# samuel-vitorino/lm.rs

Hardware: AMD Instinct MI355X
Metric: decode tok/s + %HBM-roofline, Llama-3.2-1B Q8_0 @1/2/4/8 MI355X vs CPU ref (higher is better)
Workload: dtype int8xint8->int32, f32 combine; 1 GPU; llama-3.2-1b Q8_0 (gs=128) greedy decode, 5-token synthetic prompt then 3164 tokens, batch 1; parallelism=single GPU, image_bytes=1274634496

## Files before the change

### lm.rs_amd/csrc/lmrs_kernels.hip

```cpp
#include <hip/hip_ext.h>
#include <mutex>
#include <map>
#include <set>
#include <tuple>
#include <utility>

#include "lmrs_device_math.h"
#include "lmrs_kernels.h"
#include "lmrs_stage.h"

namespace lmrs {

constexpr int kBlock = 256;
constexpr int kGS = 128;


constexpr int kMaxP = 16;

template <int NP>
__device__ __forceinline__ void rmsnorm_inplace(float4 (&v)[NP], const float4 (&wv)[NP], int n, float eps,
                                                int add_unit, float* scratch) {
    const int t = threadIdx.x;
    const int P = (n + 1023) >> 10;
    const int JP = (n >> 3) + 4;
// ... 805 lines not shown
    int best = cl;
    for (int L = cl; L <= maxL; L *= 2) {
        const int NC = L / cl;
        if (G % NC) continue;
        const int Gc = G / NC;
        if (NC > 1 && Gc > 16) continue;
        best = L;
        const int RB = (64 / L) * (kBlock / 64);
        if ((a.o + RB - 1) / RB >= 256) break;
    }
    const int NC = best / cl, Gc = G / NC;
    const int U = NC == 1 ? 16 : (Gc <= 4 ? 4 : (Gc <= 8 ? 8 : 16));
    return {best, U, NP};
}

#define LMRS_GEMV_TABLE(X)                                                                                 \
                                                                                              \
    X(8, 16, 10, PRO_PREQ, EPI_STORE, false) X(8, 16, 10, PRO_QUANT, EPI_STORE, false) X(8, 16, 10, PRO_QUANT, EPI_RESID, false) X(8, 16, 10, PRO_PREQ, EPI_RESID, false) \
    X(8, 16, 10, PRO_RMS_QUANT, EPI_STORE, false) X(8, 16, 10, PRO_RMS_QUANT, EPI_QKV, false)              \
    X(8, 16, 10, PRO_RMS_QUANT, EPI_SWIGLU, false) X(8, 16, 10, PRO_RMS_QUANT, EPI_GELU, false) X(8, 16, 10, PRO_RMS_QUANT, EPI_CLS, false) \
          \
    X(8, 16, 16, PRO_PREQ, EPI_STORE, false) X(8, 16, 16, PRO_QUANT, EPI_STORE, false) X(8, 16, 16, PRO_QUANT, EPI_RESID, false) X(8, 16, 16, PRO_PREQ, EPI_RESID, false) \
    X(4, 16, 16, PRO_PREQ, EPI_STORE, true) X(4, 16, 16, PRO_QUANT, EPI_STORE, true) X(4, 16, 16, PRO_QUANT, EPI_RESID, true) \
                                                      \
    X(32, 4, 2, PRO_RMS_QUANT, EPI_QKV, false) X(32, 4, 2, PRO_QUANT, EPI_RESID, false) X(32, 4, 2, PRO_QUANT, EPI_STORE, false) \
    X(8, 16, 2, PRO_RMS_QUANT, EPI_SWIGLU, false) X(8, 16, 2, PRO_RMS_QUANT, EPI_CLS, false) X(8, 16, 2, PRO_RMS_QUANT, EPI_QKV, false) \
    X(32, 4, 2, PRO_PREQ, EPI_STORE, false) X(8, 16, 2, PRO_PREQ, EPI_STORE, false) X(16, 8, 2, PRO_PREQ, EPI_STORE, false) \
                                              \
    X(16, 16, 4, PRO_RMS_QUANT, EPI_QKV, false) X(32, 8, 4, PRO_QUANT, EPI_RESID, false) X(16, 16, 4, PRO_QUANT, EPI_RESID, false) \
    X(8, 16, 4, PRO_RMS_QUANT, EPI_SWIGLU, false) X(8, 16, 4, PRO_RMS_QUANT, EPI_GELU, false) X(8, 16, 4, PRO_RMS_QUANT, EPI_CLS, false) \
    X(16, 16, 4, PRO_PREQ, EPI_STORE, false) X(32, 8, 4, PRO_PREQ, EPI_STORE, false)                       \
                                                                         \
    X(32, 16, 10, PRO_QUANT, EPI_RESID, false) X(32, 16, 10, PRO_QUANT, EPI_STORE, false) X(64, 16, 10, PRO_QUANT, EPI_STORE, false) \
    X(64, 16, 10, PRO_QUANT, EPI_RESID, false) X(32, 16, 10, PRO_PREQ, EPI_STORE, false) X(64, 16, 10, PRO_PREQ, EPI_STORE, false) \
                                                             \
    X(4, 16, 10, PRO_PREQ, EPI_STORE, true) X(4, 16, 10, PRO_QUANT, EPI_STORE, true) X(4, 16, 10, PRO_QUANT, EPI_RESID, true) \
    X(4, 16, 10, PRO_RMS_QUANT, EPI_STORE, true) X(4, 16, 10, PRO_RMS_QUANT, EPI_QKV, true) X(4, 16, 10, PRO_RMS_QUANT, EPI_SWIGLU, true) \
    X(4, 16, 10, PRO_RMS_QUANT, EPI_GELU, true) X(4, 16, 10, PRO_RMS_QUANT, EPI_CLS, true)                 \
    X(16, 4, 10, PRO_PREQ, EPI_STORE, true) X(16, 4, 10, PRO_QUANT, EPI_RESID, true) X(16, 4, 10, PRO_QUANT, EPI_STORE, true) \
    X(16, 4, 10, PRO_RMS_QUANT, EPI_QKV, true) X(16, 16, 10, PRO_QUANT, EPI_RESID, true) X(16, 16, 10, PRO_QUANT, EPI_STORE, true) \
    X(16, 16, 10, PRO_PREQ, EPI_STORE, true) X(8, 16, 10, PRO_PREQ, EPI_STORE, true) X(8, 16, 10, PRO_RMS_QUANT, EPI_QKV, true)

static bool gemv_instantiated(int L, int U, int NP, int pro, int epi, bool q4) {
#define X(l, u, np, p, e, q) if (L == l && U == u && NP == np && pro == p && epi == e && q4 == q) return true;
    LMRS_GEMV_TABLE(X)
#undef X
    return false;
}

static GemvShape resolve_shape(const GemvArgs& a, int pro, int epi) {
    GemvShape sh = pick_shape(a, epi);
    if (!gemv_instantiated(sh.L, sh.U, sh.NP, pro, epi, a.q4 != 0)) {
        const int big = a.n <= 10240 ? 10 : 16;
        if (gemv_instantiated(sh.L, sh.U, big, pro, epi, a.q4 != 0)) sh.NP = big;
        else sh = {a.q4 ? 4 : 8, 16, big};
    }
    return sh;
}

int gemv_grid(const GemvArgs& a, int pro, int epi) {
    const StaticClass sc = static_class(a, pro, epi);
    const GemvShape sh = sc.L ? GemvShape{sc.L, 0, 0} : resolve_shape(a, pro, epi);
    const int RB = (64 / sh.L) * ((sc.L ? sc.nt : kBlock) / 64);
    const int n_pass = (a.o + RB - 1) / RB;
    int cap = 4096;
    if (epi == EPI_CLS) cap = 512;
    else if (sc.L && (epi == EPI_SWIGLU || epi == EPI_GELU)) {
        int k = 2;
        if (n_pass / 2 > 256 && n_pass / 2 < 448 && (n_pass + 2) / 3 <= 256) k = 3;
        cap = (n_pass + k - 1) / k;
    }
    return n_pass < cap ? n_pass : cap;
}

hipError_t launch_gemv(const GemvArgs& a0, int pro, int epi, hipStream_t s, int grid_hint) {
    GemvArgs a = a0;
    a.order_barrier = a.chain_spread = 1;
    if (a.n % kGS != 0 || a.n > kMaxP * 1024 || a.o <= 0) return hipErrorInvalidValue;
    int grid = grid_hint > 0 ? grid_hint : gemv_grid(a, pro, epi);
    if (grid_hint > 0 && (epi == EPI_SWIGLU || epi == EPI_GELU)) {
        const int least = gemv_grid(a, pro, epi);
        if (grid < least) grid = least;
    }
    if (epi == EPI_CLS && a.has_tail && (!a.tail.cls_seq || !a.tail.err || !a.tail.part_pk || a.o + a.row_offset >= (1 << 20) - 1)) return hipErrorInvalidValue;
    const size_t smem = gemv_smem(a, pro);
    const StaticClass sc = static_class(a, pro, epi);
    if (sc.L) {
#define X(n_, l_, p_, e_, nt_, q_)                                                                         \
        if (a.n == n_ && sc.L == l_ && pro == p_ && epi == e_ && sc.nt == nt_ && (a.q4 != 0) == q_) {      \
            LMRS_LAUNCH_GRID((gemv_static_kernel<n_, l_, p_, e_, nt_, q_>), dim3(grid), nt_, smem, s, LMRS_HOT_OF(a), a);            \
            return hipGetLastError();                                                                      \
        }
        LMRS_STATIC_TABLE(X)
#undef X
    }
    if (pro == PRO_ADD_RMS_QUANT) return hipErrorInvalidValue;
    const GemvShape sh = resolve_shape(a, pro, epi);
#define X(l, u, np, p, e, q)                                                                               \
    if (sh.L == l && sh.U == u && sh.NP == np && pro == p && epi == e && (a.q4 != 0) == q) {              \
        LMRS_LAUNCH((gemv_kernel<l, u, np, p, e, q>), grid, smem, s, a);                                   \
        return hipGetLastError();                                                                          \
    }
    LMRS_GEMV_TABLE(X)
#undef X
    return hipErrorInvalidValue;
}

constexpr int kAttF4 = 16;

template <int HS> struct AttGeom {
    static constexpr int HS4 = HS / 4, RS = HS + 4;
    static constexpr bool ALIGNED = (kBlock % HS4 == 0) && ((16 * HS4) % kBlock == 0 || kBlock % (16 * HS4) == 0);
};
template <int HS, int NF>
__device__ __forceinline__ void att_gload(float4 (&rg)[NF], const float* __restrict__ base, int t0, int T, int CH, int kv_dim) {
    constexpr int HS4 = HS / 4;
    const int ct = (T - t0) < CH ? (T - t0) : CH, nrows = (ct + 15) & ~15, nf = nrows * HS4;
    const int r0 = (int)threadIdx.x / HS4, c4 = (int)threadIdx.x - r0 * HS4;
    const float* lane_base = base + (size_t)t0 * kv_dim + c4 * 4;
#pragma unroll
    for (int i0 = 0; i0 < NF; i0 += 4) {
        if (i0 * kBlock < nf) {
#pragma unroll
            for (int i = i0; i < i0 + 4 && i < NF; ++i) {
                int row;
                if constexpr (kBlock % HS4 == 0) row = r0 + i * (kBlock / HS4);
                else row = ((int)threadIdx.x + i * kBlock) / HS4;
                const int col4 = (kBlock % HS4 == 0) ? 0 : (((int)threadIdx.x + i * kBlock) - row * HS4 - c4) * 4;
                row = row < ct - 1 ? row : ct - 1;
                rg[i] = ld_f32x4<false>(lane_base + (size_t)row * kv_dim + col4);
            }
        }
    }
}
template <int HS, int NF, bool SCALE>
__device__ __forceinline__ void att_tstore(const float4 (&rg)[NF], float* tile, const float* rowscale, int t0, int T, int CH, int patch_t, const float* patch) {
    constexpr int HS4 = HS / 4, RS = HS + 4;
    const int ct = (T - t0) < CH ? (T - t0) : CH, nrows = (ct + 15) & ~15, nf = nrows * HS4;
    const int r0 = (int)threadIdx.x / HS4, c4 = (int)threadIdx.x - r0 * HS4;
#pragma unroll
    for (int i0 = 0; i0 < NF; i0 += 4) {
        if (i0 * kBlock < nf) {
            int row[4], col[4]; float sc[4];
#pragma unroll
            for (int u = 0; u < 4; ++u) {
                const int i = i0 + u;
                if constexpr (kBlock % HS4 == 0) { row[u] = r0 + i * (kBlock / HS4); col[u] = c4; }
                else { const int f = (int)threadIdx.x + i * kBlock; row[u] = f / HS4; col[u] = f - row[u] * HS4; }
                if constexpr (SCALE) sc[u] = rowscale[row[u] < nrows ? row[u] : nrows - 1];
            }
#pragma unroll
            for (int u = 0; u < 4; ++u) {
                const int i = i0 + u;
                if (i < NF && (AttGeom<HS>::ALIGNED || row[u] < nrows)) {
                    float4 v = rg[i];
                    if constexpr (SCALE) { v.x = sc[u] * v.x; v.y = sc[u] * v.y; v.z = sc[u] * v.z; v.w = sc[u] * v.w; }
                    *reinterpret_cast<float4*>(tile + row[u] * RS + col[u] * 4) = v;
                }
            }
        }
    }
    if (patch_t >= t0 && patch_t < t0 + ct) {
        const int fb = (patch_t - t0) * HS4, d = ((int)threadIdx.x - fb) & (kBlock - 1);
        if (d < HS4) {
            float4 v = *reinterpret_cast<const float4*>(patch + d * 4);
            if constexpr (SCALE) { const float ap = rowscale[patch_t - t0]; v.x = ap * v.x; v.y = ap * v.y; v.z = ap * v.z; v.w = ap * v.w; }
            *reinterpret_cast<float4*>(tile + (patch_t - t0) * RS + d * 4) = v;
        }
    }
}

#define ATT_STAMP(k) do { if (a.dbg && threadIdx.x == 0 && blockIdx.x == 0) a.dbg[k] = wall_clock64(); } while (0)

struct AttPre { float q0, q1, k0, k1; float2 cs; };

typedef float f32x4v __attribute__((ext_vector_type(4)));
__device__ __forceinline__ float* att_k_head(const AttnArgs& a, int kvh, int hs) {
    return a.k_cache + ((size_t)a.layer * a.n_kv_heads + kvh) * hs * (size_t)a.seq_len;
}
template <int NG>
__device__ __forceinline__ void att_kload(f32x4v (&dst)[NG], __amdgpu_buffer_rsrc_t krs, int voff, int g0, int S) {
#pragma unroll
    for (int u = 0; u < NG; ++u) {
        const auto t = __builtin_amdgcn_raw_buffer_load_b128(krs, voff, (g0 + u) * S * 16, 0);
        dst[u] = f32x4v{__uint_as_float(t[0]), __uint_as_float(t[1]), __uint_as_float(t[2]), __uint_as_float(t[3])};
    }
}
template <int NG>
__device__ __forceinline__ float att_kuse(float score, const f32x4v (&src)[NG], const float4* q4, int g0) {
#pragma unroll
    for (int u = 0; u < NG; ++u) {
        const float4 qq = q4[g0 + u];
        float pr;
        pr = qq.x * src[u].x; score = score + pr;
        pr = qq.y * src[u].y; score = score + pr;
        pr = qq.z * src[u].z; score = score + pr;
        pr = qq.w * src[u].w; score = score + pr;
    }
    return score;
}
template <int HS, int NG>
__device__ __forceinline__ float att_score_chain(f32x4v (&kk)[NG], __amdgpu_buffer_rsrc_t krs, int voff, const float* q, int S) {
    constexpr int HS4 = HS / 4;
    f32x4v kb[NG];
    float score = 0.0f;
    const float4* q4 = reinterpret_cast<const float4*>(q);
#pragma unroll
    for (int g0 = 0; g0 < HS4; g0 += 2 * NG) {
        if (g0 + NG < HS4) att_kload<NG>(kb, krs, voff, g0 + NG, S);
        score = att_kuse<NG>(score, kk, q4, g0);
        asm volatile("" : "+v"(score) : : "memory");
        if (g0 + NG < HS4) {
            if (g0 + 2 * NG < HS4) att_kload<NG>(kk, krs, voff, g0 + 2 * NG, S);
            score = att_kuse<NG>(score, kb, q4, g0 + NG);
            asm volatile("" : "+v"(score) : : "memory");
        }
    }
    return score;
}

__device__ __forceinline__ float2 rope_rotate(float v0, float v1, float fcr, float fci) {
    const float a0 = v0 * fcr, a1 = v1 * fci, b0 = v0 * fci, b1 = v1 * fcr;
    return make_float2(a0 - a1, b0 + b1);
}
__device__ __forceinline__ void k_store_pair(float* k, int S, int pos, int j, int half, float r0, float r1) {
    k[(((size_t)(j >> 2) * S + pos) << 2) + (j & 3)] = r0;
    k[(((size_t)((j + half) >> 2) * S + pos) << 2) + ((j + half) & 3)] = r1;
}
__device__ __forceinline__ float gemma_cap_window(float score, int wpos, int t) {
    score = score / 50.0f;
    score = (float)tanh((double)score);
    score = score * 50.0f;
    return score + (((unsigned)(wpos - t) <= 4096u) ? 0.0f : -2.3819763e38f);
}
template <int HS4>
__device__ __forceinline__ float tile_score(const float4* k, int ks, const float* qs) {
    constexpr int GB = 4;
    static_assert(HS4 % (2 * GB) == 0, "head size");
    const float4* q4 = reinterpret_cast<const float4*>(qs);
    auto dot = [](float score, const float4 (&q)[GB], const float4 (&kk)[GB]) __attribute__((always_inline)) {
#pragma unroll
        for (int u = 0; u < GB; ++u) {
            float pr;
            pr = q[u].x * kk[u].x; score = score + pr;
            pr = q[u].y * kk[u].y; score = score + pr;
            pr = q[u].z * kk[u].z; score = score + pr;
            pr = q[u].w * kk[u].w; score = score + pr;
        }
        return score;
    };
    float score = 0.0f;
    float4 ka[GB], qa[GB], kb[GB], qb[GB];
#pragma unroll
    for (int u = 0; u < GB; ++u) { ka[u] = k[u * ks]; qa[u] = q4[u]; }
#pragma unroll
    for (int g0 = 0; g0 < HS4; g0 += 2 * GB) {
#pragma unroll
        for (int u = 0; u < GB; ++u) { kb[u] = k[(g0 + GB + u) * ks]; qb[u] = q4[g0 + GB + u]; }
        asm volatile("" : "+v"(score) : : "memory");
        score = dot(score, qa, ka);
        if (g0 + 2 * GB < HS4) {
#pragma unroll
            for (int u = 0; u < GB; ++u) { ka[u] = k[(g0 + 2 * GB + u) * ks]; qa[u] = q4[g0 + 2 * GB + u]; }
        }
        asm volatile("" : "+v"(score) : : "memory");
        score = dot(score, qb, kb);
    }
    return score;
}
struct AttTag { const unsigned long long* gran; unsigned tag; int att_dim, kv_dim; int* err; };
template <int NG>
__device__ __forceinline__ void poll_granules(const unsigned long long* const (&gp)[NG], const AttTag& tg, int layer, unsigned long long (&xg)[NG]) {
    auto sweep = [&](unsigned long long (&x)[NG]) __attribute__((always_inline)) {
#pragma unroll
        for (int k = 0; k < NG; ++k) x[k] = __hip_atomic_load(gp[k], __ATOMIC_RELAXED, __HIP_MEMORY_SCOPE_AGENT);
    };
    auto fresh = [&](const unsigned long long (&x)[NG]) __attribute__((always_inline)) {
        bool ok = true;
#pragma unroll
        for (int k = 0; k < NG; ++k) ok = ok && (unsigned)(x[k] >> 32) == tg.tag;
        return __all(ok) != 0;
    };
    auto take = [&](const unsigned long long (&x)[NG]) __attribute__((always_inline)) {
#pragma unroll
        for (int k = 0; k < NG; ++k) xg[k] = x[k];
    };
    unsigned long long xa[NG], xb[NG];
    sweep(xa);
    for (unsigned spins = 0;; ++spins) {
        sweep(xb);
        if (fresh(xa)) { take(xa); break; }
        sweep(xa);
        if (fresh(xb)) { take(xb); break; }
        if (spins > kTagSpinMax || (spins & 1023) == 1023) {
            const int e = __hip_atomic_load(tg.err, __ATOMIC_RELAXED, __HIP_MEMORY_SCOPE_AGENT);
            if (e != 0 || spins > kTagSpinMax) {
                if (e == 0) __hip_atomic_store(tg.err, layer + 1, __ATOMIC_RELAXED, __HIP_MEMORY_SCOPE_AGENT);
                take(xb);
                break;
            }
        }
    }
}
__device__ __forceinline__ void granules_of(const AttTag& tg, int h, int kvh, int hs, int d, const unsigned long long** gp) {
    gp[0] = tg.gran + h * hs + d; gp[1] = tg.gran + tg.att_dim + kvh * hs + d; gp[2] = tg.gran + tg.att_dim + tg.kv_dim + kvh * hs + d;
}

template <int HS, int NF, bool COH, bool PRE = false, bool GEMMA = false, bool ROT = false, bool TAG = false>
__device__ __forceinline__ void attention_body(const AttnArgs& a, int h, int pos, char* smem, uint64_t etab, const AttPre& pre = AttPre(), const AttTag& tg = AttTag()) {
    static_assert(!PRE || HS / 2 <= kBlock, "one RoPE pair per lane");
    static_assert(!TAG || (HS <= kBlock && !COH && !PRE && !ROT), "granule polling: one value of each vector per lane");
    constexpr int half = HS / 2, RS = HS + 4;
    const int kv_mul = a.n_heads / a.n_kv_heads, kvh = h / kv_mul;
    const int kv_dim = a.n_kv_heads * HS;
    const int T = pos + 1;
    const int tid = threadIdx.x;
    const int CH = a.chunk;
    float* q = reinterpret_cast<float*>(smem);
    float* kn = q + HS;
    float* vn = kn + HS;
    float* red = vn + HS;
    float* tile = red + 16;
    float* att = tile + (size_t)(CH + 32) * RS;
    const size_t loff = (size_t)a.layer * a.seq_len * kv_dim;
    const int nchunks = (T + CH - 1) / CH;
    const float* vbase = a.v_cache + loff + kvh * HS;
    const int S = a.seq_len;
    float* kT = att_k_head(a, kvh, HS);
    const __amdgpu_buffer_rsrc_t krs = __builtin_amdgcn_make_buffer_rsrc(kT, 0, HS * S * 4, 0x00020000);
    constexpr int KG = HS / 4 <= 32 ? HS / 4 : 16;
    static_assert((HS / 4) % KG == 0, "head size");
    const int tc0 = tid < T ? tid : T - 1;
    f32x4v kk[KG];
    att_kload<KG>(kk, krs, tc0 * 16, 0, S);
    float4 vreg[NF];
    att_gload<HS, NF>(vreg, vbase, 0, T, CH, kv_dim);

    if constexpr (ROT) { for (int j = tid; j < HS; j += kBlock) q[j] = a.q[h * HS + j]; }
    float2 cs_tag = make_float2(0.f, 0.f);
    if constexpr (TAG) {
        cs_tag = *reinterpret_cast<const float2*>(a.rope + ((size_t)pos * half + (tid < half ? tid : 0)) * 2);
        if (tid < HS) {
            const unsigned long long* gp[3];
            unsigned long long xg[3];
            granules_of(tg, h, kvh, HS, tid, gp);
            poll_granules<3>(gp, tg, a.layer, xg);
            q[tid] = __uint_as_float((unsigned)xg[0]); kn[tid] = __uint_as_float((unsigned)xg[1]); vn[tid] = __uint_as_float((unsigned)xg[2]);
        }
        lds_barrier();
        ATT_STAMP(1);
    }
    for (int j = tid; j < (ROT ? 0 : half); j += kBlock) {
        float2 cs;
        if constexpr (PRE) cs = pre.cs; else if constexpr (TAG) cs = cs_tag; else cs = *reinterpret_cast<const float2*>(a.rope + ((size_t)pos * half + j) * 2);
        const float fcr = cs.x, fci = cs.y;
        const float q0 = TAG ? q[j] : PRE ? pre.q0 : ld_f32<COH>(a.q + h * HS + j), q1 = TAG ? q[j + half] : PRE ? pre.q1 : ld_f32<COH>(a.q + h * HS + j + half);
        const float2 rq = rope_rotate(q0, q1, fcr, fci);
        q[j] = rq.x; q[j + half] = rq.y;
        const float k0 = TAG ? kn[j] : PRE ? pre.k0 : ld_f32<COH>(a.k_raw + kvh * HS + j), k1 = TAG ? kn[j + half] : PRE ? pre.k1 : ld_f32<COH>(a.k_raw + kvh * HS + j + half);
        const float2 rk = rope_rotate(k0, k1, fcr, fci);
        kn[j] = rk.x; kn[j + half] = rk.y;
        k_store_pair(kT, S, pos, j, half, rk.x, rk.y);
        if constexpr (COH) {
            vn[j] = ld_f32<true>(vbase + (size_t)pos * kv_dim + j);
            vn[j + half] = ld_f32<true>(vbase + (size_t)pos * kv_dim + j + half);
        }
    }
    if (!TAG || HS / 4 > KG || T > kBlock) asm volatile("s_waitcnt vmcnt(0)" ::: "memory");
    lds_barrier();
    ATT_STAMP(2);
    if (!ROT && tc0 == pos) {
#pragma unroll
        for (int u = 0; u < KG; ++u) { const float4 t4 = reinterpret_cast<const float4*>(kn)[u]; kk[u] = f32x4v{t4.x, t4.y, t4.z, t4.w}; }
    }

    int wpos = pos;
    if constexpr (GEMMA) { const int wb = a.st->win_base; wpos = wb >= 0 ? wb : pos; }
    const float sqrt_hs = sqrtf((float)HS);
    float lmax = __uint_as_float(0xff800000u);
    auto finish_score = [&](float score, int t) __attribute__((always_inline)) {
        score = score / sqrt_hs;
        if constexpr (GEMMA) score = gemma_cap_window(score, wpos, t);
        if (t < T) { att[t] = score; lmax = fmaxf(lmax, score); }
    };
    finish_score(att_score_chain<HS, KG>(kk, krs, tc0 * 16, q, S), tid);
    for (int t0 = kBlock; t0 < T; t0 += kBlock) {
        const int t = t0 + tid, tc = t < T ? t : T - 1;
        f32x4v k0[KG];
        att_kload<KG>(k0, krs, tc * 16, 0, S);
        finish_score(att_score_chain<HS, KG>(k0, krs, tc * 16, q, S), t);
    }
    ATT_STAMP(4);
    lmax = wave64_max(lmax);
    if ((tid & 63) == 0) red[tid >> 6] = lmax;
    lds_barrier();
    const float mx = fmaxf(fmaxf(red[0], red[1]), fmaxf(red[2], red[3]));
    for (int t0 = 0; t0 < T; t0 += kBlock) {
        const int t = t0 + tid;
        const float e = expf_glibc_t(t < T ? att[t] - mx : 0.0f, etab);
        if (t < T) att[t] = e;
    }
    if (tid < 64) att[T + tid] = 0.0f;
    lds_barrier();
    if (tid < 64) {
        float sum = 0.0f;
        for (int t0 = 0; t0 < T; t0 += 64) {
            const int left = T - t0;
            sum = wave_serial_sum(sum, att[t0 + tid], left >= 64 ? 4 : (left + 15) >> 4);
        }
        if (tid == 0) red[4] = sum;
    }
    lds_barrier();
    const float sum = red[4];
    for (int t = tid; t < T; t += kBlock) att[t] = att[t] / sum;
    lds_barrier();
    ATT_STAMP(5);

    float o = 0.0f;
    for (int c = 0; c < nchunks; ++c) {
        const int t0 = c * CH, ct = (T - t0) < CH ? (T - t0) : CH;
        att_tstore<HS, NF, true>(vreg, tile, att + t0, t0, T, CH, (COH || TAG) ? pos : -1, vn);
        lds_barrier();
        if (c + 1 < nchunks) att_gload<HS, NF>(vreg, vbase, t0 + CH, T, CH, kv_dim);
        if (c == 0) ATT_STAMP(6);
        if (tid < HS) {
            o = serial_sum16<RS, false>(o, tile + tid, ct);
        }
        lds_barrier();
    }
    if (tid < HS) st_f32<COH>(a.out + h * HS + tid, o);
    ATT_STAMP(7);
}

template <int HS, bool GEMMA>
__global__ __launch_bounds__(kBlock) void attention_kernel(const AttnArgs a) {
    extern __shared__ __attribute__((aligned(16))) char smem[];
    const int h = blockIdx.x, kvh = h / (a.n_heads / a.n_kv_heads);
    ATT_STAMP(0);
    const uint64_t etab = exp2f_tab_lane();
    constexpr int half = HS / 2;
    const int j = threadIdx.x < half ? (int)threadIdx.x : 0;
    const int pos = a.st->pos;
    AttPre pre;
    pre.q0 = a.q[h * HS + j]; pre.q1 = a.q[h * HS + j + half];
    pre.k0 = a.k_raw[kvh * HS + j]; pre.k1 = a.k_raw[kvh * HS + j + half];
    pre.cs = *reinterpret_cast<const float2*>(a.rope + ((size_t)pos * half + j) * 2);
    ATT_STAMP(1);
    attention_body<HS, kAttF4, false, true, GEMMA>(a, h, pos, smem, etab, pre);
}

static size_t attention_smem(int head_size, int chunk, int seq_len) {
    return (size_t)(3 * head_size + 16 + (size_t)(chunk + 32) * (head_size + 4) + ((seq_len + 3) & ~3) + 64) * 4;
}

int attention_chunk(int head_size) {
    int ch = (16384 / head_size) & ~31;
    if (ch > 256) ch = 256;
    return ch < 32 ? 32 : ch;
}

template <int HS, bool GEMMA>
static hipError_t launch_attention_hsg(const AttnArgs& a, size_t smem, hipStream_t s) {
    allow_big_lds(reinterpret_cast<const void*>(attention_kernel<HS, GEMMA>));
    LMRS_LAUNCH_GRID((attention_kernel<HS, GEMMA>), dim3(a.n_heads), kBlock, smem, s, a);
    return hipGetLastError();
}
template <int HS>
static hipError_t launch_attention_hs(const AttnArgs& a, size_t smem, hipStream_t s) {
    return a.gemma ? launch_attention_hsg<HS, true>(a, smem, s) : launch_attention_hsg<HS, false>(a, smem, s);
}

hipError_t launch_attention(const AttnArgs& a0, hipStream_t s) {
    AttnArgs a = a0;
    a.chunk = attention_chunk(a.head_size);
    if (a.chunk * (a.head_size / 4) > kAttF4 * kBlock) return hipErrorInvalidValue;
    const size_t smem = attention_smem(a.head_size, a.chunk, a.seq_len);
    switch (a.head_size) {
        case 64: return launch_attention_hs<64>(a, smem, s);
        case 96: return launch_attention_hs<96>(a, smem, s);
        case 128: return launch_attention_hs<128>(a, smem, s);
        case 256: return launch_attention_hs<256>(a, smem, s);
        default: return hipErrorInvalidValue;
    }
}

template <int HS> struct WaveGeom {
    static constexpr int HS4 = HS / 4, ND = (HS + 63) / 64, NH2 = (HS / 2 + 63) / 64;
    static constexpr int TW = HS <= 64 ? 128 : 64;
    static constexpr int NPASS = TW / 64;
    static constexpr size_t SMEM = (size_t)(2 * HS + TW + 16) * 4 + (size_t)HS4 * TW * 16;
};
constexpr int qa_wave_T(int hs) { return hs == 64 ? 64 * 4 : ((hs == 96 || hs == 128) ? 128 : 0); }

template <int HS, bool GEMMA>
__device__ __forceinline__ void attention_wave_tag(const AttnArgs& a, const int h, const int pos, char* smem, const uint64_t etab, const AttTag& tg) {
    using W = WaveGeom<HS>;
    constexpr int HS4 = W::HS4, ND = W::ND, NH2 = W::NH2, TW = W::TW, NPASS = W::NPASS, half = HS / 2;
    const int lane = threadIdx.x & 63;
    const int kv_mul = a.n_heads / a.n_kv_heads, kvh = h / kv_mul, kv_dim = a.n_kv_heads * HS;
    const int T = pos + 1, S = a.seq_len;
    float* qs = reinterpret_cast<float*>(smem);
    float* kn = qs + HS;
    float* att = kn + HS;
    float4* kt = reinterpret_cast<float4*>(att + TW + 16);
    float* kT = att_k_head(a, kvh, HS);
    const float* vbase = a.v_cache + (size_t)a.layer * S * kv_dim + kvh * HS;
    if (a.dbg && lane == 0 && blockIdx.x == 0) a.dbg[0] = wall_clock64();

    float2 cs[NH2];
#pragma unroll
    for (int i = 0; i < NH2; ++i) { const int j = lane + 64 * i; cs[i] = *reinterpret_cast<const float2*>(a.rope + ((size_t)pos * half + (j < half ? j : 0)) * 2); }
#pragma unroll
    for (int p = 0; p < NPASS; ++p) {
        if (64 * p < pos) {
#pragma unroll
            for (int g = 0; g < HS4; ++g)
                __builtin_amdgcn_global_load_lds((const LMRS_GLOBAL void*)(kT + ((size_t)g * S + 64 * p + lane) * 4),
                                                 (__attribute__((address_space(3))) void*)(kt + g * TW + 64 * p), 16, 0, 0);
        }
    }
    float v[ND][TW];
    const __amdgpu_buffer_rsrc_t vrs = __builtin_amdgcn_make_buffer_rsrc(const_cast<float*>(vbase), 0, 0x7fffffff, 0x00020000);
    const int vrow = kv_dim * 4;
    auto vblock = [&](auto self, auto t0c) __attribute__((always_inline)) -> void {
        constexpr int t0 = decltype(t0c)::value;
        if constexpr (t0 < TW) {
            if (t0 < pos) {
#pragma unroll
                for (int u = 0; u < 16; ++u)
#pragma unroll
                    for (int i = 0; i < ND; ++i) {
                        const int d = lane + 64 * i;
                        v[i][t0 + u] = __uint_as_float(__builtin_amdgcn_raw_buffer_load_b32(vrs, (d < HS ? d : 0) * 4, (t0 + u) * vrow, 0));
                    }
                self(self, std::integral_constant<int, t0 + 16>());
            }
        }
    };
    vblock(vblock, std::integral_constant<int, 0>());
#pragma unroll
    for (int t = 0; t < TW; ++t)
#pragma unroll
        for (int i = 0; i < ND; ++i) { v[i][t] = t < pos ? v[i][t] : 0.0f; asm volatile("" : "+v"(v[i][t])); }
    if (a.dbg && lane == 0 && blockIdx.x == 0) a.dbg[1] = wall_clock64();

    unsigned long long xg[3 * ND];
    {
        const unsigned long long* gp[3 * ND];
#pragma unroll
        for (int i = 0; i < ND; ++i) { const int d = lane + 64 * i; granules_of(tg, h, kvh, HS, d < HS ? d : 0, gp + 3 * i); }
        poll_granules<3 * ND>(gp, tg, a.layer, xg);
    }
    asm volatile("s_waitcnt vmcnt(0)" ::: "memory");
    if (a.dbg && lane == 0 && blockIdx.x == 0) a.dbg[2] = wall_clock64();
    float vnew[ND];
#pragma unroll
    for (int i = 0; i < ND; ++i) {
        const int d = lane + 64 * i;
        vnew[i] = __uint_as_float((unsigned)xg[3 * i + 2]);
        if (d < HS) { qs[d] = __uint_as_float((unsigned)xg[3 * i]); kn[d] = __uint_as_float((unsigned)xg[3 * i + 1]); }
    }
#pragma unroll
    for (int i = 0; i < NH2; ++i) {
        const int j = lane + 64 * i;
        if (j < half) {
            const float2 rq = rope_rotate(qs[j], qs[j + half], cs[i].x, cs[i].y);
            qs[j] = rq.x; qs[j + half] = rq.y;
            const float2 rk = rope_rotate(kn[j], kn[j + half], cs[i].x, cs[i].y);
            k_store_pair(kT, S, pos, j, half, rk.x, rk.y);
            k_store_pair(reinterpret_cast<float*>(kt), TW, pos, j, half, rk.x, rk.y);
        }
    }
    if (a.dbg && lane == 0 && blockIdx.x == 0) a.dbg[3] = wall_clock64();

    int wpos = pos;
    if constexpr (GEMMA) { const int wb = a.st->win_base; wpos = wb >= 0 ? wb : pos; }
    const float sqrt_hs = sqrtf((float)HS), ninf = __uint_as_float(0xff800000u);
    float sc[NPASS];
    float lmax = ninf;
#pragma unroll
    for (int p = 0; p < NPASS; ++p) {
        sc[p] = ninf;
        if (64 * p < T) {
            const int t = 64 * p + lane;
            float score = tile_score<HS4>(kt + t, TW, qs) / sqrt_hs;
            if constexpr (GEMMA) score = gemma_cap_window(score, wpos, t);
            sc[p] = t < T ? score : ninf;
            lmax = fmaxf(lmax, sc[p]);
        }
    }
    if (a.dbg && lane == 0 && blockIdx.x == 0) a.dbg[4] = wall_clock64();
    const float mx = wave64_max(lmax);
    float ex[NPASS];
#pragma unroll
    for (int p = 0; p < NPASS; ++p) {
        ex[p] = 0.0f;
        if (64 * p < T) {
            const int t = 64 * p + lane;
            const float e = expf_glibc_t(t < T ? sc[p] - mx : 0.0f, etab);
            ex[p] = t < T ? e : 0.0f;
        }
    }
    float sum = 0.0f;
#pragma unroll
    for (int p = 0; p < NPASS; ++p) {
        if (64 * p < T) {
            const int left = T - 64 * p;
            sum = wave_serial_sum(sum, ex[p], left >= 64 ? 4 : (left + 15) >> 4);
        }
    }
    float ap_lane = 0.0f;
#pragma unroll
    for (int p = 0; p < NPASS; ++p) {
        if (64 * p < T) {
            const int t = 64 * p + lane;
            const float w = ex[p] / sum;
            att[t] = t < pos ? w : 0.0f;
            if ((pos >> 6) == p) ap_lane = w;
        }
    }
    const float a_pos = __builtin_bit_cast(float, __builtin_amdgcn_readlane(__builtin_bit_cast(int, ap_lane), pos & 63));
    if (a.dbg && lane == 0 && blockIdx.x == 0) a.dbg[5] = wall_clock64();
    float o[ND];
#pragma unroll
    for (int i = 0; i < ND; ++i) o[i] = 0.0f;
#pragma unroll
    for (int t0 = 0; t0 < TW; t0 += 16) {
        if (t0 < pos) {
            float4 w4[4];
#pragma unroll
            for (int u = 0; u < 4; ++u) w4[u] = reinterpret_cast<const float4*>(att)[t0 / 4 + u];
#pragma unroll
            for (int u = 0; u < 4; ++u)
#pragma unroll
                for (int i = 0; i < ND; ++i) {
                    float pr;
                    pr = w4[u].x * v[i][t0 + 4 * u + 0]; o[i] = o[i] + pr;
                    pr = w4[u].y * v[i][t0 + 4 * u + 1]; o[i] = o[i] + pr;
                    pr = w4[u].z * v[i][t0 + 4 * u + 2]; o[i] = o[i] + pr;
                    pr = w4[u].w * v[i][t0 + 4 * u + 3]; o[i] = o[i] + pr;
                }
        }
    }
#pragma unroll
    for (int i = 0; i < ND; ++i) {
        const int d = lane + 64 * i;
        const float pr = a_pos * vnew[i];
        o[i] = o[i] + pr;
        if (d < HS) a.out[h * HS + d] = o[i];
    }
    if (a.dbg && lane == 0 && blockIdx.x == 0) a.dbg[7] = wall_clock64();
}

constexpr size_t kPairSmem = (size_t)(2 * 2 * 64 + 128 + 16 + 16) * 4 + (size_t)16 * 128 * 16 + (size_t)64 * 64 * 4;
template <bool GEMMA>
__device__ __forceinline__ void attention_pair_tag(const AttnArgs& a, const int h, const int pos, char* smem, const uint64_t etab, const AttTag& tg) {
    constexpr int HS = 64, HS4 = 16, TW = 128, half = 32;
    const int lane = threadIdx.x & 63, wv = __builtin_amdgcn_readfirstlane((int)threadIdx.x >> 6);
    const bool two = pos >= 64;
    if (wv > (two ? 1 : 0)) return;
    const int tb = two ? 64 * wv : 0;
    const int kv_mul = a.n_heads / a.n_kv_heads, kvh = h / kv_mul, kv_dim = a.n_kv_heads * HS;
    const int T = pos + 1, S = a.seq_len;
    float* base = reinterpret_cast<float*>(smem);
    float* qs = base + wv * 2 * HS;
    float* kn = qs + HS;
    float* att = base + 4 * HS;
    float* red = att + TW + 16;
    float4* kt = reinterpret_cast<float4*>(red + 16);
    float* prod = reinterpret_cast<float*>(kt + HS4 * TW);
    float* kT = att_k_head(a, kvh, HS);
    const float* vbase = a.v_cache + (size_t)a.layer * S * kv_dim + kvh * HS;
    if (a.dbg && lane == 0 && wv == 0 && blockIdx.x == 0) a.dbg[0] = wall_clock64();

    const float2 cs = *reinterpret_cast<const float2*>(a.rope + ((size_t)pos * half + (lane < half ? lane : 0)) * 2);
    if (tb < pos) {
#pragma unroll
        for (int g = 0; g < HS4; ++g)
            __builtin_amdgcn_global_load_lds((const LMRS_GLOBAL void*)(kT + ((size_t)g * S + tb + lane) * 4),
                                             (__attribute__((address_space(3))) void*)(kt + g * TW + tb), 16, 0, 0);
    }
    float v[64];
    const __amdgpu_buffer_rsrc_t vrs = __builtin_amdgcn_make_buffer_rsrc(const_cast<float*>(vbase), 0, 0x7fffffff, 0x00020000);
    const int vrow = kv_dim * 4, vb0 = tb * vrow;
    auto vblock = [&](auto self, auto u0c) __attribute__((always_inline)) -> void {
        constexpr int u0 = decltype(u0c)::value;
        if constexpr (u0 < 64) {
            if (tb + u0 < pos) {
#pragma unroll
                for (int u = 0; u < 16; ++u) v[u0 + u] = __uint_as_float(__builtin_amdgcn_raw_buffer_load_b32(vrs, lane * 4, vb0 + (u0 + u) * vrow, 0));
                self(self, std::integral_constant<int, u0 + 16>());
            }
        }
    };
    vblock(vblock, std::integral_constant<int, 0>());
#pragma unroll
    for (int u = 0; u < 64; ++u) { v[u] = tb + u < pos ? v[u] : 0.0f; asm volatile("" : "+v"(v[u])); }
    if (a.dbg && lane == 0 && wv == 0 && blockIdx.x == 0) a.dbg[1] = wall_clock64();

    unsigned long long xg[3];
    {
        const unsigned long long* gp[3];
        granules_of(tg, h, kvh, HS, lane, gp);
        poll_granules<3>(gp, tg, a.layer, xg);
    }
    asm volatile("s_waitcnt vmcnt(0)" ::: "memory");
    if (a.dbg && lane == 0 && wv == 0 && blockIdx.x == 0) a.dbg[2] = wall_clock64();
    const float vnew = __uint_as_float((unsigned)xg[2]);
    qs[lane] = __uint_as_float((unsigned)xg[0]); kn[lane] = __uint_as_float((unsigned)xg[1]);
    if (lane < half) {
        const int j = lane;
        const float2 rq = rope_rotate(qs[j], qs[j + half], cs.x, cs.y);
        qs[j] = rq.x; qs[j + half] = rq.y;
        const float2 rk = rope_rotate(kn[j], kn[j + half], cs.x, cs.y);
        if (wv == 0) k_store_pair(kT, S, pos, j, half, rk.x, rk.y);
        if ((pos >> 6) == (two ? wv : 0)) k_store_pair(reinterpret_cast<float*>(kt), TW, pos, j, half, rk.x, rk.y);
    }
    if (a.dbg && lane == 0 && wv == 0 && blockIdx.x == 0) a.dbg[3] = wall_clock64();

    int wpos = pos;
    if constexpr (GEMMA) { const int wb = a.st->win_base; wpos = wb >= 0 ? wb : pos; }
    const float sqrt_hs = sqrtf((float)HS), ninf = __uint_as_float(0xff800000u);
    const int t = tb + lane;
    float sc;
    {
        float score = tile_score<HS4>(kt + t, TW, qs) / sqrt_hs;
        if constexpr (GEMMA) score = gemma_cap_window(score, wpos, t);
        sc = t < T ? score : ninf;
    }
    if (a.dbg && lane == 0 && wv == 0 && blockIdx.x == 0) a.dbg[4] = wall_clock64();
    float mx = wave64_max(sc);
    if (two) {
        if (lane == 0) red[wv] = mx;
        lds_barrier();
        mx = fmaxf(red[0], red[1]);
    }
    const float e0 = expf_glibc_t(t < T ? sc - mx : 0.0f, etab);
    const float ex = t < T ? e0 : 0.0f;
    float sum;
    if (!two) {
        sum = wave_serial_sum(0.0f, ex, (T + 15) >> 4);
    } else {
        if (wv == 0) { sum = wave_serial_sum(0.0f, ex, 4); if (lane == 0) red[2] = sum; }
        lds_barrier();
        if (wv == 1) { sum = wave_serial_sum(red[2], ex, (T - 64 + 15) >> 4); if (lane == 0) red[3] = sum; }
        lds_barrier();
        sum = red[3];
    }
    const float w = ex / sum;
    att[t] = t < pos ? w : 0.0f;
    const bool own_pos = (pos >> 6) == (two ? wv : 0);
    float a_pos = 0.0f;
    if (own_pos) a_pos = __builtin_bit_cast(float, __builtin_amdgcn_readlane(__builtin_bit_cast(int, w), pos & 63));
    if (a.dbg && lane == 0 && wv == 0 && blockIdx.x == 0) a.dbg[5] = wall_clock64();
    if (two && wv == 1) {
        if (lane == 0) red[4] = a_pos;
#pragma unroll
        for (int u0 = 0; u0 < 64; u0 += 16) {
            if (64 + u0 < pos) {
                float4 w4[4];
#pragma unroll
                for (int u = 0; u < 4; ++u) w4[u] = reinterpret_cast<const float4*>(att)[(64 + u0) / 4 + u];
#pragma unroll
                for (int u = 0; u < 4; ++u) {
                    prod[(u0 + 4 * u + 0) * HS + lane] = w4[u].x * v[u0 + 4 * u + 0];
                    prod[(u0 + 4 * u + 1) * HS + lane] = w4[u].y * v[u0 + 4 * u + 1];
                    prod[(u0 + 4 * u + 2) * HS + lane] = w4[u].z * v[u0 + 4 * u + 2];
                    prod[(u0 + 4 * u + 3) * HS + lane] = w4[u].w * v[u0 + 4 * u + 3];
                }
            }
        }
        lds_barrier();
        return;
    }
    float o = 0.0f;
#pragma unroll
    for (int u0 = 0; u0 < 64; u0 += 16) {
        if (u0 < pos) {
            float4 w4[4];
#pragma unroll
            for (int u = 0; u < 4; ++u) w4[u] = reinterpret_cast<const float4*>(att)[u0 / 4 + u];
#pragma unroll
            for (int u = 0; u < 4; ++u) {
                float pr;
                pr = w4[u].x * v[u0 + 4 * u + 0]; o = o + pr;
                pr = w4[u].y * v[u0 + 4 * u + 1]; o = o + pr;
                pr = w4[u].z * v[u0 + 4 * u + 2]; o = o + pr;
                pr = w4[u].w * v[u0 + 4 * u + 3]; o = o + pr;
            }
        }
    }
    if (two) {
        lds_barrier();
        a_pos = red[4];
#pragma unroll
        for (int u0 = 0; u0 < 64; u0 += 16) {
            if (64 + u0 < pos) {
                float pb[16];
#pragma unroll
                for (int u = 0; u < 16; ++u) pb[u] = prod[(u0 + u) * HS + lane];
#pragma unroll
                for (int u = 0; u < 16; ++u) o = o + pb[u];
            }
        }
    }
    {
        const float pr = a_pos * vnew;
        o = o + pr;
        a.out[h * HS + lane] = o;
    }
    if (a.dbg && lane == 0 && wv == 0 && blockIdx.x == 0) a.dbg[7] = wall_clock64();
}

constexpr int kMultiWaves = 4;
constexpr size_t kMultiSmem = (size_t)(kMultiWaves * 2 * 64 + 64 * kMultiWaves + 16 + 32) * 4 + (size_t)(kMultiWaves - 1) * 64 * 64 * 4;
template <bool GEMMA>
__device__ __forceinline__ void attention_multi_tag(const AttnArgs& a, const int h, const int pos, char* smem, const uint64_t etab, const AttTag& tg) {
    constexpr int HS = 64, HS4 = 16, half = 32;
    const int lane = threadIdx.x & 63, wv = __builtin_amdgcn_readfirstlane((int)threadIdx.x >> 6);
    const int nw = (pos >> 6) + 1 < kMultiWaves ? (pos >> 6) + 1 : kMultiWaves;
    if (wv >= nw) return;
    const int tb = 64 * wv, t = tb + lane;
    const int kv_mul = a.n_heads / a.n_kv_heads, kvh = h / kv_mul, kv_dim = a.n_kv_heads * HS;
    const int T = pos + 1, S = a.seq_len;
    float* base = reinterpret_cast<float*>(smem);
    float* qs = base + wv * 2 * HS;
    float* kn = qs + HS;
    float* att = base + kMultiWaves * 2 * HS;
    float* red = att + 64 * kMultiWaves + 16;
    float* prod = red + 32;
    float* kT = att_k_head(a, kvh, HS);
    const float* vbase = a.v_cache + (size_t)a.layer * S * kv_dim + kvh * HS;
    if (a.dbg && lane == 0 && wv == 0 && blockIdx.x == 0) a.dbg[0] = wall_clock64();

    const float2 cs = *reinterpret_cast<const float2*>(a.rope + ((size_t)pos * half + (lane < half ? lane : 0)) * 2);
    f32x4v kreg[HS4];
    {
        const int tk = t < S ? t : S - 1;
        if (tb < pos) {
#pragma unroll
            for (int g = 0; g < HS4; ++g) kreg[g] = *reinterpret_cast<const f32x4v*>(kT + ((size_t)g * S + tk) * 4);
        } else {
#pragma unroll
            for (int g = 0; g < HS4; ++g) kreg[g] = f32x4v{0.0f, 0.0f, 0.0f, 0.0f};
        }
    }
    float v[64];
    const __amdgpu_buffer_rsrc_t vrs = __builtin_amdgcn_make_buffer_rsrc(const_cast<float*>(vbase), 0, 0x7fffffff, 0x00020000);
    const int vrow = kv_dim * 4;
    auto vblock = [&](auto self, auto u0c) __attribute__((always_inline)) -> void {
        constexpr int u0 = decltype(u0c)::value;
        if constexpr (u0 < 64) {
            if (tb + u0 < pos) {
#pragma unroll
                for (int u = 0; u < 16; ++u) {
                    const int row = tb + u0 + u < S ? tb + u0 + u : S - 1;
                    v[u0 + u] = __uint_as_float(__builtin_amdgcn_raw_buffer_load_b32(vrs, lane * 4, row * vrow, 0));
                }
                self(self, std::integral_constant<int, u0 + 16>());
            }
        }
    };
    vblock(vblock, std::integral_constant<int, 0>());
#pragma unroll
    for (int u = 0; u < 64; ++u) { v[u] = tb + u < pos ? v[u] : 0.0f; asm volatile("" : "+v"(v[u])); }
    if (a.dbg && lane == 0 && wv == 0 && blockIdx.x == 0) a.dbg[1] = wall_clock64();

    unsigned long long xg[3];
    {
        const unsigned long long* gp[3];
        granules_of(tg, h, kvh, HS, lane, gp);
        poll_granules<3>(gp, tg, a.layer, xg);
    }
    asm volatile("s_waitcnt vmcnt(0)" ::: "memory");
    if (a.dbg && lane == 0 && wv == 0 && blockIdx.x == 0) a.dbg[2] = wall_clock64();
    const float vnew = __uint_as_float((unsigned)xg[2]);
    qs[lane] = __uint_as_float((unsigned)xg[0]); kn[lane] = __uint_as_float((unsigned)xg[1]);
    const bool own_pos = (pos >> 6) == wv;
    if (lane < half) {
        const int j = lane;
        const float2 rq = rope_rotate(qs[j], qs[j + half], cs.x, cs.y);
        qs[j] = rq.x; qs[j + half] = rq.y;
        const float2 rk = rope_rotate(kn[j], kn[j + half], cs.x, cs.y);
        kn[j] = rk.x; kn[j + half] = rk.y;
        if (wv == 0) k_store_pair(kT, S, pos, j, half, rk.x, rk.y);
    }
    if (own_pos) {
#pragma unroll
        for (int g = 0; g < HS4; ++g) {
            const float4 n4 = reinterpret_cast<const float4*>(kn)[g];
            const bool me = lane == (pos & 63);
            kreg[g][0] = me ? n4.x : kreg[g][0]; kreg[g][1] = me ? n4.y : kreg[g][1]; kreg[g][2] = me ? n4.z : kreg[g][2]; kreg[g][3] = me ? n4.w : kreg[g][3];
        }
    }
    if (a.dbg && lane == 0 && wv == 0 && blockIdx.x == 0) a.dbg[3] = wall_clock64();

    int wpos = pos;
    if constexpr (GEMMA) { const int wb = a.st->win_base; wpos = wb >= 0 ? wb : pos; }
    const float sqrt_hs = sqrtf((float)HS), ninf = __uint_as_float(0xff800000u);
    float sc;
    {
        float score = 0.0f;
#pragma unroll
        for (int g = 0; g < HS4; ++g) {
            const float4 q4 = reinterpret_cast<const float4*>(qs)[g];
            float pr;
            pr = q4.x * kreg[g][0]; score = score + pr;
            pr = q4.y * kreg[g][1]; score = score + pr;
            pr = q4.z * kreg[g][2]; score = score + pr;
            pr = q4.w * kreg[g][3]; score = score + pr;
        }
        score = score / sqrt_hs;
        if constexpr (GEMMA) score = gemma_cap_window(score, wpos, t);
        sc = t < T ? score : ninf;
    }
    if (a.dbg && lane == 0 && wv == 0 && blockIdx.x == 0) a.dbg[4] = wall_clock64();
    float mx = wave64_max(sc);
    if (nw > 1) {
        if (lane == 0) red[wv] = mx;
        lds_barrier();
        mx = red[0];
        for (int w = 1; w < nw; ++w) mx = fmaxf(mx, red[w]);
    }
    const float e0 = expf_glibc_t(t < T ? sc - mx : 0.0f, etab);
    const float ex = t < T ? e0 : 0.0f;
    float sum;
    if (nw == 1) {
        sum = wave_serial_sum(0.0f, ex, (T + 15) >> 4);
    } else {
        for (int s = 0; s < nw; ++s) {
            if (wv == s) {
                const int left = T - 64 * s;
                const float part = wave_serial_sum(s ? red[8 + s - 1] : 0.0f, ex, left >= 64 ? 4 : (left + 15) >> 4);
                if (lane == 0) red[8 + s] = part;
            }
            lds_barrier();
        }
        sum = red[8 + nw - 1];
    }
    const float w = ex / sum;
    att[t] = t < pos ? w : 0.0f;
    float a_pos = 0.0f;
    if (own_pos) a_pos = __builtin_bit_cast(float, __builtin_amdgcn_readlane(__builtin_bit_cast(int, w), pos & 63));
    if (a.dbg && lane == 0 && wv == 0 && blockIdx.x == 0) a.dbg[5] = wall_clock64();
    if (wv > 0) {
        if (own_pos && lane == 0) red[4] = a_pos;
        float* mine = prod + (size_t)(wv - 1) * 64 * HS;
#pragma unroll
        for (int u0 = 0; u0 < 64; u0 += 16) {
            if (tb + u0 < pos) {
                float4 w4[4];
#pragma unroll
                for (int u = 0; u < 4; ++u) w4[u] = reinterpret_cast<const float4*>(att)[(tb + u0) / 4 + u];
#pragma unroll
                for (int u = 0; u < 4; ++u) {
                    mine[(u0 + 4 * u + 0) * HS + lane] = w4[u].x * v[u0 + 4 * u + 0];
                    mine[(u0 + 4 * u + 1) * HS + lane] = w4[u].y * v[u0 + 4 * u + 1];
                    mine[(u0 + 4 * u + 2) * HS + lane] = w4[u].z * v[u0 + 4 * u + 2];
                    mine[(u0 + 4 * u + 3) * HS + lane] = w4[u].w * v[u0 + 4 * u + 3];
                }
            }
        }
        lds_barrier();
        return;
    }
    float o = 0.0f;
#pragma unroll
    for (int u0 = 0; u0 < 64; u0 += 16) {
        if (u0 < pos) {
            float4 w4[4];
#pragma unroll
            for (int u = 0; u < 4; ++u) w4[u] = reinterpret_cast<const float4*>(att)[u0 / 4 + u];
#pragma unroll
            for (int u = 0; u < 4; ++u) {
                float pr;
                pr = w4[u].x * v[u0 + 4 * u + 0]; o = o + pr;
                pr = w4[u].y * v[u0 + 4 * u + 1]; o = o + pr;
                pr = w4[u].z * v[u0 + 4 * u + 2]; o = o + pr;
                pr = w4[u].w * v[u0 + 4 * u + 3]; o = o + pr;
            }
        }
    }
    if (nw > 1) {
        lds_barrier();
        a_pos = red[4];
        for (int k0 = 0; k0 < 64 * (kMultiWaves - 1); k0 += 16) {
            if (64 + k0 < pos) {
                float pb[16];
#pragma unroll
                for (int u = 0; u < 16; ++u) pb[u] = prod[(k0 + u) * HS + lane];
#pragma unroll
                for (int u = 0; u < 16; ++u) o = o + pb[u];
            }
        }
    }
    {
        const float pr = a_pos * vnew;
        o = o + pr;
        a.out[h * HS + lane] = o;
    }
    if (a.dbg && lane == 0 && wv == 0 && blockIdx.x == 0) a.dbg[7] = wall_clock64();
}

template <int HS> struct QuadGeom {
    static constexpr int HS4 = HS / 4, ND = (HS + 63) / 64, NH2 = (HS / 2 + 63) / 64;
    static constexpr int KPW = HS <= 128 ? 32 : 16, TWK = 4 * KPW;
    static constexpr int NPASS = TWK / 64;
    static constexpr size_t SMEM = (size_t)(4 * 2 * HS + TWK + 16 + 32) * 4 + (size_t)HS4 * TWK * 16;
    static_assert((size_t)3 * KPW * ND * 64 * 4 <= (size_t)HS4 * TWK * 16, "the products alias the K tile");
};
template <int HS, bool GEMMA>
__device__ __forceinline__ void attention_quad_tag(const AttnArgs& a, const int h, const int pos, char* smem, const uint64_t etab, const AttTag& tg) {
    using Q = QuadGeom<HS>;
    constexpr int HS4 = Q::HS4, ND = Q::ND, NH2 = Q::NH2, KPW = Q::KPW, TWK = Q::TWK, half = HS / 2;
    const int lane = threadIdx.x & 63, wv = __builtin_amdgcn_readfirstlane((int)threadIdx.x >> 6);
    const int kpw = (KPW == 32 && pos >= 64) ? 32 : 16;
    const int tb = kpw * wv;
    const int kv_mul = a.n_heads / a.n_kv_heads, kvh = h / kv_mul, kv_dim = a.n_kv_heads * HS;
    const int T = pos + 1, S = a.seq_len;
    float* base = reinterpret_cast<float*>(smem);
    float* qs = base + wv * 2 * HS;
    float* kn = qs + HS;
    float* att = base + 4 * 2 * HS;
    float* red = att + TWK + 16;
    float4* kt = reinterpret_cast<float4*>(red + 32);
    float* prod = reinterpret_cast<float*>(kt);
    float* kT = att_k_head(a, kvh, HS);
    const float* vbase = a.v_cache + (size_t)a.layer * S * kv_dim + kvh * HS;
    if (a.dbg && lane == 0 && wv == 0 && blockIdx.x == 0) a.dbg[0] = wall_clock64();

    float2 cs[NH2];
#pragma unroll
    for (int i = 0; i < NH2; ++i) { const int j = lane + 64 * i; cs[i] = *reinterpret_cast<const float2*>(a.rope + ((size_t)pos * half + (j < half ? j : 0)) * 2); }
#pragma unroll
    for (int p = 0; p < Q::NPASS; ++p) {
        if (64 * p < pos) {
#pragma unroll
            for (int gg = 0; gg < HS4 / 4; ++gg) {
                const int g = wv * (HS4 / 4) + gg;
                __builtin_amdgcn_global_load_lds((const LMRS_GLOBAL void*)(kT + ((size_t)g * S + 64 * p + lane) * 4),
                                                 (__attribute__((address_space(3))) void*)(kt + g * TWK + 64 * p), 16, 0, 0);
            }
        }
    }
    float v[ND][KPW];
    const __amdgpu_buffer_rsrc_t vrs = __builtin_amdgcn_make_buffer_rsrc(const_cast<float*>(vbase), 0, 0x7fffffff, 0x00020000);
    const int vrow = kv_dim * 4, vb0 = tb * vrow;
    auto vblock = [&](auto self, auto u0c) __attribute__((always_inline)) -> void {
        constexpr int u0 = decltype(u0c)::value;
        if constexpr (u0 < KPW) {
            if (u0 < kpw && tb + u0 < pos) {
#pragma unroll
// ... 1028 lines not shown
```

Before: 1328 tok/s.

## Split attention granule polling across waves with pipelined asm poll loop

Replaces the generic granule poll in the pair-tag attention path with an inline-assembly loop that keeps two or three load sweeps in flight and checks tags with scalar compares. Polling is also split by wave: wave 0 waits only on q, while wave 1 waits on k and v, applies RoPE through permlane32 swaps, and writes the new key to LDS and the global cache. Short sequences now use the otherwise idle second wave to prefetch K tiles and handle k/v. The aim is to cut handoff latency between the producing QKV stage and attention. In exchange it adds a barrier, hand-written asm with its own spin limit, and deferred vmcnt drains.

Result: no change. 1319 tok/s, median of 2 (-0.7%).

```diff
diff --git a/lm.rs_amd/csrc/lmrs_kernels.hip b/lm.rs_amd/csrc/lmrs_kernels.hip
--- a/lm.rs_amd/csrc/lmrs_kernels.hip
+++ b/lm.rs_amd/csrc/lmrs_kernels.hip
@@ -1131,6 +1131,76 @@
         }
     }
 }
+#ifndef LMRS_Q_SWEEPS
+#define LMRS_Q_SWEEPS 3
+#endif
+constexpr int kQSweeps = LMRS_Q_SWEEPS;
+static_assert(kQSweeps == 2 || kQSweeps == 3, "poll_counted: two or three sweeps in flight");
+struct QPoll { unsigned long long x00, x01, x02, x10, x11, x12, x20, x21, x22; };
+#define LMRS_QP_LD1(s) "global_load_dwordx2 %[x" #s "0], %[p0], off sc1\n\t"
+#define LMRS_QP_LD2(s) LMRS_QP_LD1(s) "global_load_dwordx2 %[x" #s "1], %[p1], off sc1\n\t"
+#define LMRS_QP_LD3(s) LMRS_QP_LD2(s) "global_load_dwordx2 %[x" #s "2], %[p2], off sc1\n\t"
+#define LMRS_QP_EQ(s, g) "v_lshrrev_b64 %[t], 32, %[x" #s #g "]\n\tv_cmp_eq_u64_e32 vcc, %[tag], %[t]\n\t"
+#define LMRS_QP_CK1(s) LMRS_QP_EQ(s, 0) "s_mov_b64 %[acc], vcc\n\t"
+#define LMRS_QP_CK2(s) LMRS_QP_CK1(s) LMRS_QP_EQ(s, 1) "s_and_b64 %[acc], %[acc], vcc\n\t"
+#define LMRS_QP_CK3(s) LMRS_QP_CK2(s) LMRS_QP_EQ(s, 2) "s_and_b64 %[acc], %[acc], vcc\n\t"
+#define LMRS_QP_OUT1(s) "v_mov_b64_e32 %[o0], %[x" #s "0]\n\t"
+#define LMRS_QP_OUT2(s) LMRS_QP_OUT1(s) "v_mov_b64_e32 %[o1], %[x" #s "1]\n\t"
+#define LMRS_QP_OUT3(s) LMRS_QP_OUT2(s) "v_mov_b64_e32 %[o2], %[x" #s "2]\n\t"
+#define LMRS_QP_STEP(n, s, snew, w, l) LMRS_QP_LD##n(snew) "s_waitcnt vmcnt(" #w ")\n\t" LMRS_QP_CK##n(s) "s_cmp_eq_u64 %[acc], exec\n\ts_cbranch_scc1 " #l "f\n\t"
+#define LMRS_QP_FOUND(n, s, l) #l ":\n\t" LMRS_QP_OUT##n(s) "s_mov_b32 %[ok], 1\n\ts_branch 9f\n"
+#define LMRS_QP_AGAIN(n, s) "s_sub_u32 %[n], %[n], 1\n\ts_cmp_lg_u32 %[n], 0\n\ts_cbranch_scc1 1b\n\ts_waitcnt vmcnt(0)\n\t" LMRS_QP_OUT##n(s) "s_mov_b32 %[ok], 0\n\ts_branch 9f\n"
+#define LMRS_QP_LOOP3(n, w) LMRS_QP_LD##n(0) LMRS_QP_LD##n(1) "s_movk_i32 %[n], 341\n1:\n\t" LMRS_QP_STEP(n, 0, 2, w, 2) LMRS_QP_STEP(n, 1, 0, w, 3) \
+    LMRS_QP_STEP(n, 2, 1, w, 4) LMRS_QP_AGAIN(n, 1) LMRS_QP_FOUND(n, 0, 2) LMRS_QP_FOUND(n, 1, 3) LMRS_QP_FOUND(n, 2, 4) "9:\n\t"
+#define LMRS_QP_LOOP2(n, w) LMRS_QP_LD##n(0) "s_movk_i32 %[n], 512\n1:\n\t" LMRS_QP_STEP(n, 0, 1, w, 2) LMRS_QP_STEP(n, 1, 0, w, 3) \
+    LMRS_QP_AGAIN(n, 0) LMRS_QP_FOUND(n, 0, 2) LMRS_QP_FOUND(n, 1, 3) "9:\n\t"
+#define LMRS_QP_ASM(loop) asm volatile(loop \
+    : [x00] "=&v"(xq.x00), [x01] "=&v"(xq.x01), [x02] "=&v"(xq.x02), [x10] "=&v"(xq.x10), [x11] "=&v"(xq.x11), [x12] "=&v"(xq.x12),                   \
+      [x20] "=&v"(xq.x20), [x21] "=&v"(xq.x21), [x22] "=&v"(xq.x22), [t] "=&v"(t), [o0] "=&v"(o0), [o1] "=&v"(o1), [o2] "=&v"(o2),                   \
+      [acc] "=&s"(acc), [ok] "=&s"(ok), [n] "=&s"(n)                                                                                               \
+    : [p0] "v"(gp[0]), [p1] "v"(gp[NG > 1 ? 1 : 0]), [p2] "v"(gp[NG > 2 ? 2 : 0]), [tag] "s"(tag64) : "vcc", "scc", "memory")
+template <int NG>
+__device__ __forceinline__ void poll_counted(const unsigned long long* const (&gp)[NG], const AttTag& tg, int layer, unsigned (&val)[NG], QPoll& xq) {
+    static_assert(NG >= 1 && NG <= 3, "q, k, v");
+    const unsigned long long tag64 = tg.tag;
+    unsigned long long o0 = 0, o1 = 0, o2 = 0, t, acc;
+    for (unsigned rounds = 0;; ++rounds) {
+        int ok, n;
+        if constexpr (kQSweeps == 3) {
+            if constexpr (NG == 1) LMRS_QP_ASM(LMRS_QP_LOOP3(1, 2)); else if constexpr (NG == 2) LMRS_QP_ASM(LMRS_QP_LOOP3(2, 4)); else LMRS_QP_ASM(LMRS_QP_LOOP3(3, 6));
+        } else {
+            if constexpr (NG == 1) LMRS_QP_ASM(LMRS_QP_LOOP2(1, 1)); else if constexpr (NG == 2) LMRS_QP_ASM(LMRS_QP_LOOP2(2, 2)); else LMRS_QP_ASM(LMRS_QP_LOOP2(3, 3));
+        }
+        if (ok) break;
+        const int e = __hip_atomic_load(tg.err, __ATOMIC_RELAXED, __HIP_MEMORY_SCOPE_AGENT);
+        if (e != 0 || rounds >= kTagSpinMax / 1024) {
+            if (e == 0) __hip_atomic_store(tg.err, layer + 1, __ATOMIC_RELAXED, __HIP_MEMORY_SCOPE_AGENT);
+            break;
+        }
+    }
+    val[0] = (unsigned)o0;
+    if constexpr (NG > 1) val[1] = (unsigned)o1;
+    if constexpr (NG > 2) val[2] = (unsigned)o2;
+}
+#undef LMRS_QP_ASM
+#undef LMRS_QP_LOOP2
+#undef LMRS_QP_LOOP3
+#undef LMRS_QP_AGAIN
+#undef LMRS_QP_FOUND
+#undef LMRS_QP_STEP
+#undef LMRS_QP_OUT3
+#undef LMRS_QP_OUT2
+#undef LMRS_QP_OUT1
+#undef LMRS_QP_CK3
+#undef LMRS_QP_CK2
+#undef LMRS_QP_CK1
+#undef LMRS_QP_EQ
+#undef LMRS_QP_LD3
+#undef LMRS_QP_LD2
+#undef LMRS_QP_LD1
+__device__ __forceinline__ void poll_drain(QPoll& xq) {
+    asm volatile("s_waitcnt vmcnt(0)" : "+v"(xq.x00), "+v"(xq.x01), "+v"(xq.x02), "+v"(xq.x10), "+v"(xq.x11), "+v"(xq.x12), "+v"(xq.x20), "+v"(xq.x21), "+v"(xq.x22) : : "memory");
+}
 __device__ __forceinline__ void granules_of(const AttTag& tg, int h, int kvh, int hs, int d, const unsigned long long** gp) {
     gp[0] = tg.gran + h * hs + d; gp[1] = tg.gran + tg.att_dim + kvh * hs + d; gp[2] = tg.gran + tg.att_dim + tg.kv_dim + kvh * hs + d;
 }
@@ -1487,13 +1557,13 @@
     constexpr int HS = 64, HS4 = 16, TW = 128, half = 32;
     const int lane = threadIdx.x & 63, wv = __builtin_amdgcn_readfirstlane((int)threadIdx.x >> 6);
     const bool two = pos >= 64;
-    if (wv > (two ? 1 : 0)) return;
+    if (wv > 1) return;
     const int tb = two ? 64 * wv : 0;
     const int kv_mul = a.n_heads / a.n_kv_heads, kvh = h / kv_mul, kv_dim = a.n_kv_heads * HS;
     const int T = pos + 1, S = a.seq_len;
     float* base = reinterpret_cast<float*>(smem);
     float* qs = base + wv * 2 * HS;
-    float* kn = qs + HS;
+    float* vn = base + HS;
     float* att = base + 4 * HS;
     float* red = att + TW + 16;
     float4* kt = reinterpret_cast<float4*>(red + 16);
@@ -1502,8 +1572,37 @@
     const float* vbase = a.v_cache + (size_t)a.layer * S * kv_dim + kvh * HS;
     if (a.dbg && lane == 0 && wv == 0 && blockIdx.x == 0) a.dbg[0] = wall_clock64();
 
-    const float2 cs = *reinterpret_cast<const float2*>(a.rope + ((size_t)pos * half + (lane < half ? lane : 0)) * 2);
-    if (tb < pos) {
+    const float2 cs = *reinterpret_cast<const float2*>(a.rope + ((size_t)pos * half + (lane & 31)) * 2);
+    auto rotate = [&](unsigned raw) __attribute__((always_inline)) {
+        const auto sw = __builtin_amdgcn_permlane32_swap(raw, raw, false, false);
+        const float2 r = rope_rotate(__uint_as_float(sw[0]), __uint_as_float(sw[1]), cs.x, cs.y);
+        return lane < half ? r.x : r.y;
+    };
+    const size_t kslot = ((size_t)(lane >> 2) * TW + pos) * 4 + (lane & 3), kcell = ((size_t)(lane >> 2) * S + pos) * 4 + (lane & 3);
+    const unsigned long long* gp[3];
+    granules_of(tg, h, kvh, HS, lane, gp);
+
+    if (!two && wv == 1) {
+        if (0 < pos) {
+#pragma unroll
+            for (int g = 0; g < HS4; ++g)
+                __builtin_amdgcn_global_load_lds((const LMRS_GLOBAL void*)(kT + ((size_t)g * S + lane) * 4),
+                                                 (__attribute__((address_space(3))) void*)(kt + g * TW), 16, 0, 0);
+        }
+        const unsigned long long* gkv[2] = {gp[1], gp[2]};
+        unsigned xkv[2];
+        QPoll xk{};
+        __builtin_amdgcn_s_waitcnt(0x0f70);
+        poll_counted<2>(gkv, tg, a.layer, xkv, xk);
+        const float kr = rotate(xkv[0]);
+        reinterpret_cast<float*>(kt)[kslot] = kr;
+        vn[lane] = __uint_as_float(xkv[1]);
+        lds_barrier();
+        kT[kcell] = kr;
+        poll_drain(xk);
+        return;
+    }
+    if (two) {
 #pragma unroll
         for (int g = 0; g < HS4; ++g)
             __builtin_amdgcn_global_load_lds((const LMRS_GLOBAL void*)(kT + ((size_t)g * S + tb + lane) * 4),
@@ -1527,24 +1626,26 @@
     for (int u = 0; u < 64; ++u) { v[u] = tb + u < pos ? v[u] : 0.0f; asm volatile("" : "+v"(v[u])); }
     if (a.dbg && lane == 0 && wv == 0 && blockIdx.x == 0) a.dbg[1] = wall_clock64();
 
-    unsigned long long xg[3];
-    {
-        const unsigned long long* gp[3];
-        granules_of(tg, h, kvh, HS, lane, gp);
-        poll_granules<3>(gp, tg, a.layer, xg);
-    }
-    asm volatile("s_waitcnt vmcnt(0)" ::: "memory");
+    unsigned qraw;
+    QPoll xq{};
+    __builtin_amdgcn_s_waitcnt(0x0f70);
+    if (wv == 0) {
+        const unsigned long long* gq[1] = {gp[0]};
+        unsigned xv[1];
+        poll_counted<1>(gq, tg, a.layer, xv, xq);
+        qraw = xv[0];
+    } else {
+        unsigned xv[3];
+        poll_counted<3>(gp, tg, a.layer, xv, xq);
+        qraw = xv[0];
+        const float kr = rotate(xv[1]);
+        reinterpret_cast<float*>(kt)[kslot] = kr;
+        kT[kcell] = kr;
+        vn[lane] = __uint_as_float(xv[2]);
+    }
     if (a.dbg && lane == 0 && wv == 0 && blockIdx.x == 0) a.dbg[2] = wall_clock64();
-    const float vnew = __uint_as_float((unsigned)xg[2]);
-    qs[lane] = __uint_as_float((unsigned)xg[0]); kn[lane] = __uint_as_float((unsigned)xg[1]);
-    if (lane < half) {
-        const int j = lane;
-        const float2 rq = rope_rotate(qs[j], qs[j + half], cs.x, cs.y);
-        qs[j] = rq.x; qs[j + half] = rq.y;
-        const float2 rk = rope_rotate(kn[j], kn[j + half], cs.x, cs.y);
-        if (wv == 0) k_store_pair(kT, S, pos, j, half, rk.x, rk.y);
-        if ((pos >> 6) == (two ? wv : 0)) k_store_pair(reinterpret_cast<float*>(kt), TW, pos, j, half, rk.x, rk.y);
-    }
+    qs[lane] = rotate(qraw);
+    if (!two) lds_barrier();
     if (a.dbg && lane == 0 && wv == 0 && blockIdx.x == 0) a.dbg[3] = wall_clock64();
 
     int wpos = pos;
@@ -1577,6 +1678,8 @@
         sum = red[3];
     }
     const float w = ex / sum;
+    poll_drain(xq);
+    const float vnew = vn[lane];
     att[t] = t < pos ? w : 0.0f;
     const bool own_pos = (pos >> 6) == (two ? wv : 0);
     float a_pos = 0.0f;
```
